# rpng/suo_slam

Measured on AMD Instinct MI355X. Metric: frames/sec (obj-crops/sec) YCB-V 640x480 8-obj; ADD(-S) vs ref, higher is better.
Workload: dtype f32 (2 x fp16 split products)

## Files before the change

### suo_slam_amd/build.py

```python
from __future__ import annotations

import os
import subprocess
import sys

HERE = os.path.dirname(os.path.abspath(__file__))
CSRC = os.path.join(HERE, "csrc")
LIB = os.path.join(HERE, "libsuo_hip.so")
SOURCES = ["capi.hip", "net.hip", "net_weights.hip", "conv.hip", "conv_wino.hip", "conv_wino_x3.hip", "conv_small.hip", "stem_x3.hip", "res_small.hip", "res_small_x3.hip", "gemm_persist.hip", "gemm_bf16x3.hip", "misc.hip", "calibrate.hip", "pnp.hip", "lm.hip", "lm_big.hip", "lm_cam.hip", "lm_cam2.hip", "lm_frame.hip", "lm_frame2.hip", "lm_dist.hip", "pose_cov.hip", "pose_cov_graph.hip", "resid_stats.hip", "track_cov.hip", "ba_comm.hip", "pnp_api.hip", "ba_stage.hip", "ba_api.hip", "ba_ctx.hip", "ba_drive.hip", "cov_stage.hip", "pose_cov_api.hip", "track_cov_api.hip", "frame_geom.hip", "eval.hip", "eval_bop.hip", "eval_nees.hip", "eval_nees_api.hip", "raster.hip", "eval_vsd.hip", "gt_info.hip", "gt_info_api.hip", "slam_score.hip", "slam_vote.hip"]
HIPCC = os.environ.get("HIPCC", "/opt/rocm/bin/hipcc")
FLAGS = ["--offload-arch=gfx950", "-O3", "-std=c++17", "-fPIC", "-ffp-contract=off"]


def _stale(target, deps):
    if not os.path.exists(target):
        return True
    t = os.path.getmtime(target)
    return any(os.path.getmtime(d) > t for d in deps)


def build(force: bool = False, verbose: bool = True) -> str:
    srcs = [os.path.join(CSRC, s) for s in SOURCES if os.path.exists(os.path.join(CSRC, s))]
    hdrs = [os.path.join(CSRC, f) for f in os.listdir(CSRC) if f.endswith(".h")]
    hdrs.append(os.path.join(os.path.dirname(HERE), "include", "suo_hip.h"))
    objs = []
    procs = []
    for src in srcs:
        obj = src[:-4] + ".o"
        objs.append(obj)
        deps = [src] + hdrs
        if src.endswith("lm_big.hip"):
            deps.append(os.path.join(CSRC, "lm.hip"))
        if force or _stale(obj, deps):
            cmd = [HIPCC] + FLAGS + ["-c", src, "-o", obj]
            if verbose:
                print(" ".join(cmd), flush=True)
            procs.append((src, subprocess.Popen(cmd)))
    for src, p in procs:
        if p.wait() != 0:
            raise RuntimeError(f"hipcc failed on {src}")
    if force or procs or _stale(LIB, objs):
        cmd = [HIPCC, "--offload-arch=gfx950", "-shared", "-fPIC", "-o", LIB] + objs + ["-ldl"]
        if verbose:
            print(" ".join(cmd), flush=True)
        subprocess.check_call(cmd)
    return LIB


if __name__ == "__main__":
    build(force="--force" in sys.argv)
    print(LIB)
```

### suo_slam_amd/csrc/conv_wino_x3.hip

```cpp
#include <string.h>

#include "bf16x3.h"
#include "f16x2.h"
#include "buffer_ops.h"
#include "suo_internal.h"
#include "tune.h"

namespace suo {

typedef float x_f32x4 __attribute__((ext_vector_type(4)));
typedef float x_f32x16 __attribute__((ext_vector_type(16)));
typedef unsigned x_u32x2 __attribute__((ext_vector_type(2)));
typedef unsigned x_u32x4 __attribute__((ext_vector_type(4)));
typedef __bf16 x_bf16x8 __attribute__((ext_vector_type(8)));
typedef _Float16 x_f16x8 __attribute__((ext_vector_type(8)));

__device__ __forceinline__ x_f32x16 x_mfma32(float a, float b, x_f32x16 c) { return __builtin_amdgcn_mfma_f32_32x32x2f32(a, b, c, 0, 0, 0); }
__device__ __forceinline__ int x_acc_row(int r, int lane) { return (r & 3) + 8 * (r >> 2) + 4 * (lane >> 5); }

__device__ __forceinline__ x_f32x4 x_sub4(x_f32x4 a, x_f32x4 b) { return a - b; }
__device__ __forceinline__ x_f32x4 x_add4(x_f32x4 a, x_f32x4 b) { return a + b; }
__device__ __forceinline__ void x_add16(x_f32x16& z, const x_f32x16& t) { z += t; }
__device__ __forceinline__ void x_sub16(x_f32x16& z, const x_f32x16& t) { z -= t; }

constexpr int X_CK = 16, X_PKH = 20, X_TH = 8, X_TW = 16, X_IH = 10, X_IW = 18, X_NPIX = X_IH * X_IW;

void pack_wino_weight_bf16x3(const float* W, int N, int C, int Np, int Cp, const float* out_scale, uint16_t* out) {
    static const double G[4][3] = {{1, 0, 0}, {0.5, 0.5, 0.5}, {0.5, -0.5, 0.5}, {0, 0, 1}};
    const int NB = Np / 32;
    memset(out, 0, (size_t)Np * Cp * 16 * 3 * sizeof(uint16_t));
    for (int n = 0; n < N; ++n)
        for (int c = 0; c < C; ++c) {
            const float* g = W + ((size_t)n * C + c) * 9;
            const double sc = out_scale ? (double)out_scale[n] : 1.0;
            double Gg[4][3], U[4][4];
            for (int i = 0; i < 4; ++i)
                for (int j = 0; j < 3; ++j) Gg[i][j] = G[i][0] * g[j] + G[i][1] * g[3 + j] + G[i][2] * g[6 + j];
            for (int i = 0; i < 4; ++i)
                for (int j = 0; j < 4; ++j) U[i][j] = (Gg[i][0] * G[j][0] + Gg[i][1] * G[j][1] + Gg[i][2] * G[j][2]) * sc;
            const int chunk = c / X_CK, cc = c % X_CK, nb = n / 32, lane = (cc / 8) * 32 + (n % 32), e = cc % 8;
            for (int comp = 0; comp < 16; ++comp) {
                uint16_t t[3];
                s3_split_host((float)(comp >= 12 ? -U[comp >> 2][comp & 3] : U[comp >> 2][comp & 3]), t);
                for (int p = 0; p < 3; ++p) out[((((size_t)(chunk * 16 + comp) * NB + nb) * 3 + p) * 64 + lane) * 8 + e] = t[p];
            }
        }
}

void pack_tail_weight_bf16x3(const float* W3, int N2, int K, uint16_t* out) {
    const int NB = N2 / 32;
    for (int n = 0; n < N2; ++n)
        for (int k = 0; k < K; ++k) {
            const int ks = k / 16, kk = k % 16, lane = (kk / 8) * 32 + (n % 32), e = kk % 8, nb = n / 32;
            uint16_t t[3];
            s3_split_host(W3[(size_t)n * K + k], t);
            for (int p = 0; p < 3; ++p) out[((((size_t)(ks * NB + nb) * 3 + p) * 64 + lane) * 8) + e] = t[p];
        }
}

void pack_wino_weight_f16x2(const float* W, int N, int C, int Np, int Cp, const float* out_scale, uint16_t* out, float* oscale_out) {
    static const double G[4][3] = {{1, 0, 0}, {0.5, 0.5, 0.5}, {0.5, -0.5, 0.5}, {0, 0, 1}};
    const int NB = Np / 32;
    memset(out, 0, (size_t)Np * Cp * 16 * 2 * sizeof(uint16_t));
    for (int n = 0; n < Np; ++n) oscale_out[n] = ldexpf(1.f, -S2_XSHIFT);
    float* Un = (float*)malloc((size_t)C * 16 * sizeof(float));
    for (int n = 0; n < N; ++n) {
        float mx = 0.f;
        for (int c = 0; c < C; ++c) {
            const float* g = W + ((size_t)n * C + c) * 9;
            const double sc = out_scale ? (double)out_scale[n] : 1.0;
            double Gg[4][3];
            for (int i = 0; i < 4; ++i)
                for (int j = 0; j < 3; ++j) Gg[i][j] = G[i][0] * g[j] + G[i][1] * g[3 + j] + G[i][2] * g[6 + j];
            for (int i = 0; i < 4; ++i)
                for (int j = 0; j < 4; ++j) {
                    const float u = (float)((Gg[i][0] * G[j][0] + Gg[i][1] * G[j][1] + Gg[i][2] * G[j][2]) * sc);
                    Un[c * 16 + i * 4 + j] = i == 3 ? -u : u;
                    mx = fmaxf(mx, fabsf(u));
                }
        }
        const int t = s2_row_shift(mx);
        oscale_out[n] = ldexpf(1.f, -(t + S2_XSHIFT));
        for (int c = 0; c < C; ++c) {
            const int chunk = c / X_CK, cc = c % X_CK, nb = n / 32, lane = (cc / 8) * 32 + (n % 32), e = cc % 8;
            for (int comp = 0; comp < 16; ++comp) {
                uint16_t h[2];
                s2_split_host(ldexpf(Un[c * 16 + comp], t), h);
                for (int p = 0; p < 2; ++p) out[((((size_t)(chunk * 16 + comp) * NB + nb) * 2 + p) * 64 + lane) * 8 + e] = h[p];
            }
        }
    }
    free(Un);
}

void pack_tail_weight_f16x2(const float* W3, int N2, int K, uint16_t* out, float* oscale_out) { pack_gemm_weight_f16x2(W3, N2, K, out, oscale_out); }

template <bool FUSE, bool UP = false, bool TX3 = false, int NT = 4, int NP = 3, bool NEXT = false, bool W8 = false>
__global__ __launch_bounds__(W8 ? 512 : 256) __attribute__((amdgpu_waves_per_eu(2))) void wino3x3_x3_kernel(const ConvArgs a) {
    static_assert(NT == 4 || (NT == 2 && !FUSE), "64-channel form: plain convolution only");
    static_assert(!W8 || (NT == 4 && NP == 2 && !NEXT && (TX3 || !FUSE)), "eight waves: the fp16 form of the 128-channel kernel, without the next block's conv1");
    constexpr int NTHR = W8 ? 512 : 256;
    static_assert(!NEXT || (FUSE && TX3 && NP == 2), "the next block's conv1 rides on the fp16 tail");
    static_assert(NP == 3 || !FUSE || TX3, "the fp16 form's tail runs on the fp16 pipe");
    constexpr int HSZ = X_NPIX * X_PKH;
    constexpr int VROW = 16;
    constexpr int VPL = 16 * 32 * VROW;
    constexpr int VFLOATS = NP * VPL / 2;
    constexpr int TAILF = NP * 8 * (64 * 32 + 32) / 4;
    constexpr int SFLOATS = W8 ? (2 * HSZ + VFLOATS > TAILF + 8 * 32 * 36 ? 2 * HSZ + VFLOATS : TAILF + 8 * 32 * 36) : 2 * HSZ + VFLOATS;
    __shared__ __attribute__((aligned(16))) float S[SFLOATS];
    float (*Hin)[HSZ] = reinterpret_cast<float (*)[HSZ]>(&S[0]);
    uint16_t* V = reinterpret_cast<uint16_t*>(&S[2 * HSZ]);
    const int tid = threadIdx.x, lane = tid & 63;
    const int w = __builtin_amdgcn_readfirstlane(tid >> 6);
    const int tiles_x = (a.OW + X_TW - 1) / X_TW, tiles_y = (a.OH + X_TH - 1) / X_TH;
    int bid = blockIdx.x;
    if ((gridDim.x & 7) == 0) bid = (bid & 7) * (gridDim.x >> 3) + (bid >> 3);
    const int l = bid / (tiles_x * tiles_y);
    bid -= l * tiles_x * tiles_y;
    const int ty0 = bid / tiles_x, tx0 = bid - ty0 * tiles_x;
    const int oy0 = ty0 * X_TH, ox0 = tx0 * X_TW;
    const int iy0 = oy0 - 1, ix0 = ox0 - 1;
    const int nch = a.C / X_CK;
    const float* in_l = a.in + (size_t)l * a.H * a.W * a.C;
    const __amdgpu_buffer_rsrc_t in_srd = make_srd(in_l, (size_t)a.H * a.W * a.C * sizeof(float));
    const __amdgpu_buffer_rsrc_t w_srd = make_srd(a.Wp, (size_t)a.N * a.C * 16 * NP * sizeof(uint16_t));
    const __amdgpu_buffer_rsrc_t out_srd = make_srd(a.out + (size_t)l * a.OH * a.OW * a.N, (size_t)a.OH * a.OW * a.N * sizeof(float));

    constexpr int NF4 = X_NPIX * 4, NLD = (NF4 + NTHR - 1) / NTHR;
    int avoff[NLD];
#pragma unroll
    for (int i = 0; i < NLD; ++i) {
        const int idx = tid + i * NTHR;
        const int pix = idx >> 2, cc = idx & 3;
        const int py = pix / X_IW, px = pix - py * X_IW;
        const int iy = iy0 + py, ix = ix0 + px;
        const bool ok = idx < NF4 && iy >= 0 && iy < a.H && ix >= 0 && ix < a.W;
        avoff[i] = ok ? ((iy * a.W + ix) * a.C + cc * 4) * 4 : BUF_OOB;
    }
    x_f32x4 areg[NLD];
    auto gload = [&](int c) {
#pragma unroll
        for (int i = 0; i < NLD; ++i) areg[i] = buf_load(in_srd, avoff[i], c * X_CK * 4);
    };
    float dmax = 0.f;
    const float xs = NP == 2 ? s2_xscale(a.xscale) : 1.f;
    auto sstore = [&](int buf) {
#pragma unroll
        for (int i = 0; i < NLD; ++i) {
            const int idx = tid + i * NTHR;
            if constexpr (NP == 2) {
                areg[i] *= xs;
                dmax = s2_track(s2_track(dmax, areg[i][0], areg[i][1]), areg[i][2], areg[i][3]);
            }
            if (idx < NF4) *(x_f32x4*)&Hin[buf][(idx >> 2) * X_PKH + (idx & 3) * 4] = areg[i];
        }
    };
    const int wvoff = lane * 16;
    const int wn = NT == 4 ? (W8 ? (w & 3) : w) : (w & 1), wc = NT == 4 ? (W8 ? (w >> 2) : 0) : (w >> 1);
    constexpr bool HALF = NT == 2 || W8;
    constexpr int NPAIR = HALF ? 4 : 8;
    const int wsbase = wn * NP * 1024;
    auto bload = [&](int gc, x_u32x4 (&b)[NP]) {
        const int g = gc;
#pragma unroll
        for (int p = 0; p < NP; ++p) b[p] = __builtin_bit_cast(x_u32x4, buf_load(w_srd, wvoff + p * 1024, g * (NT * NP * 1024) + wsbase));
    };
    const int tt = tid & 31, tq = (tid >> 5) & 3, th = (tid >> 7) & 1;
    const int tv = __builtin_amdgcn_readfirstlane(tid >> 8);
    const int t_ty = tt >> 3, t_tx = tt & 7;
    const int hbase = ((2 * t_ty + th) * X_IW + 2 * t_tx) * X_PKH + tq * 4;
    const int vbase = tt * VROW + ((((tq >> 1) ^ (((tt >> 2) ^ (tt >> 3)) & 1)) * 8) + (tq & 1) * 4);
    auto vstore = [&](int comp, x_f32x4 v) {
        if constexpr (NP == 2) {
            const unsigned h0 = s2_pack_rn(v[0], v[1]), h1 = s2_pack_rn(v[2], v[3]);
            *(x_u32x2*)&V[comp * 32 * VROW + vbase] = x_u32x2{h0, h1};
            const unsigned l0 = s2_lo_pack(v[0], v[1], h0), l1 = s2_lo_pack(v[2], v[3], h1);
            *(x_u32x2*)&V[VPL + comp * 32 * VROW + vbase] = x_u32x2{l0, l1};
            return;
        }
#pragma unroll
        for (int p = 0; p < 3; ++p) {
            const unsigned q0 = s3_pack_rn(v[0], v[1]), q1 = s3_pack_rn(v[2], v[3]);
            *(x_u32x2*)&V[p * VPL + comp * 32 * VROW + vbase] = x_u32x2{q0, q1};
            if (p < 2) {
                v = x_sub4(v, x_f32x4{s3_lo(q0), s3_hi(q0), s3_lo(q1), s3_hi(q1)});
            }
        }
    };
    const int hother = th ? 0 : 2 * X_IW * X_PKH;
    const float hsign = th ? -1.f : 1.f;
    auto transform = [&](int buf) {
        const float* hs = &Hin[buf][hbase];
        if constexpr (W8) {
            const int xi = tv == 0 ? (th ? 3 : 0) : (th ? 2 : 1);
            x_f32x4 e[4];
#pragma unroll
            for (int c = 0; c < 4; ++c) {
                if (tv == 0) {
                    e[c] = x_sub4(*(const x_f32x4*)(hs + c * X_PKH), *(const x_f32x4*)(hs + (2 * X_IW + c) * X_PKH));
                } else {
                    const x_f32x4 l1 = *(const x_f32x4*)(hs + (X_IW + c) * X_PKH), lx = *(const x_f32x4*)(hs + hother + c * X_PKH);
                    e[c] = x_f32x4{__builtin_fmaf(lx[0], hsign, l1[0]), __builtin_fmaf(lx[1], hsign, l1[1]), __builtin_fmaf(lx[2], hsign, l1[2]), __builtin_fmaf(lx[3], hsign, l1[3])};
                }
            }
            vstore(xi * 4 + 0, x_sub4(e[0], e[2]));
            vstore(xi * 4 + 1, x_add4(e[1], e[2]));
            vstore(xi * 4 + 2, x_sub4(e[2], e[1]));
            vstore(xi * 4 + 3, x_sub4(e[1], e[3]));
            return;
        }
        x_f32x4 L0[4], L1[4], L2[4], Lx[4];
#pragma unroll
        for (int c = 0; c < 4; ++c) {
            L0[c] = *(const x_f32x4*)(hs + c * X_PKH);
            L1[c] = *(const x_f32x4*)(hs + (X_IW + c) * X_PKH);
            L2[c] = *(const x_f32x4*)(hs + (2 * X_IW + c) * X_PKH);
            Lx[c] = *(const x_f32x4*)(hs + hother + c * X_PKH);
        }
        x_f32x4 eA[4], eB[4];
#pragma unroll
        for (int c = 0; c < 4; ++c) {
            eA[c] = x_sub4(L0[c], L2[c]);
            eB[c] = x_f32x4{__builtin_fmaf(Lx[c][0], hsign, L1[c][0]), __builtin_fmaf(Lx[c][1], hsign, L1[c][1]), __builtin_fmaf(Lx[c][2], hsign, L1[c][2]),
                            __builtin_fmaf(Lx[c][3], hsign, L1[c][3])};
        }
        const int xiA = th ? 3 : 0, xiB = th ? 2 : 1;
        vstore(xiA * 4 + 0, x_sub4(eA[0], eA[2]));
        vstore(xiA * 4 + 1, x_add4(eA[1], eA[2]));
        vstore(xiA * 4 + 2, x_sub4(eA[2], eA[1]));
        vstore(xiA * 4 + 3, x_sub4(eA[1], eA[3]));
        vstore(xiB * 4 + 0, x_sub4(eB[0], eB[2]));
        vstore(xiB * 4 + 1, x_add4(eB[1], eB[2]));
        vstore(xiB * 4 + 2, x_sub4(eB[2], eB[1]));
        vstore(xiB * 4 + 3, x_sub4(eB[1], eB[3]));
    };

    x_f32x16 zero16;
#pragma unroll
    for (int r = 0; r < 16; ++r) zero16[r] = 0.f;
    x_f32x16 out[4], Z[8];
#pragma unroll
    for (int p = 0; p < 4; ++p)
#pragma unroll
        for (int r = 0; r < 16; ++r) out[p][r] = 0.f;
#pragma unroll
    for (int p = 0; p < 8; ++p)
#pragma unroll
        for (int r = 0; r < 16; ++r) Z[p][r] = 0.f;
    auto mac6 = [&](x_f32x16& acc, const x_bf16x8 (&f)[NP], const x_u32x4 (&bw)[NP], bool from_zero) {
        if constexpr (NP == 2) {
            constexpr int UI[3] = {0, 1, 0}, UJ[3] = {1, 0, 0};
#pragma unroll
            for (int t = 0; t < 3; ++t)
                acc = __builtin_amdgcn_mfma_f32_32x32x16_f16(__builtin_bit_cast(x_f16x8, f[UI[t]]), __builtin_bit_cast(x_f16x8, bw[UJ[t]]), (t == 0 && from_zero) ? zero16 : acc, 0, 0, 0);
            return;
        }
        constexpr int TI[6] = {0, 1, 2, 0, 1, 0}, TJ[6] = {2, 1, 0, 1, 0, 0};
#pragma unroll
        for (int t = 0; t < 6; ++t)
            acc = __builtin_amdgcn_mfma_f32_32x32x16_bf16(f[TI[t] % NP], __builtin_bit_cast(x_bf16x8, bw[TJ[t] % NP]), (t == 0 && from_zero) ? zero16 : acc, 0, 0, 0);
    };
    auto comp_of = [&](int pair, int which) -> int {
        if (!HALF) return pair < 4 ? (which ? 12 + pair : pair) : (which ? 8 + (pair - 4) : 4 + (pair - 4));
        return wc * 8 + 2 * pair + which;
    };
    const int afoff = (lane & 31) * VROW + (((lane >> 5) ^ (((lane >> 2) ^ (lane >> 3)) & 1)) * 8);
    x_u32x4 bring[2][2][NP];
    gload(0);
    bload(comp_of(0, 0), bring[0][0]);
    bload(comp_of(0, 1), bring[0][1]);
    sstore(0);
    __syncthreads();

#ifdef SUO_WX3_PROF
    long long pt[5] = {0, 0, 0, 0, 0}, p0 = clock64();
#define XPROF(i) do { const long long _t = clock64(); pt[i] += _t - p0; p0 = _t; } while (0)
#else
#define XPROF(i) do { } while (0)
#endif
    for (int c = 0; c < nch; ++c) {
        const int buf = c & 1;
        const bool more = c + 1 < nch;
        if (more) gload(c + 1);
        transform(buf);
        XPROF(0);
        __syncthreads();
        XPROF(1);
        if (more) sstore(buf ^ 1);
        XPROF(2);
#pragma unroll
        for (int pair = 0; pair < NPAIR; ++pair) {
            const int slot = pair & 1;
            {
                const int np = pair + 1 < NPAIR ? pair + 1 : 0, nc = pair + 1 < NPAIR ? c : (more ? c + 1 : c);
                bload(nc * 16 + comp_of(np, 0), bring[slot ^ 1][0]);
                bload(nc * 16 + comp_of(np, 1), bring[slot ^ 1][1]);
            }
            const int ca = comp_of(pair, 0), cb = comp_of(pair, 1);
            x_bf16x8 afa[NP], afb[NP];
#pragma unroll
            for (int p = 0; p < NP; ++p) {
                afa[p] = *(const x_bf16x8*)&V[p * VPL + ca * 32 * VROW + afoff];
                afb[p] = *(const x_bf16x8*)&V[p * VPL + cb * 32 * VROW + afoff];
            }
            __builtin_amdgcn_sched_barrier(0);
            if (HALF) {
                mac6(Z[2 * pair], afa, bring[slot][0], false);
                mac6(Z[2 * pair + 1], afb, bring[slot][1], false);
            } else if (pair < 4) {
                mac6(Z[pair], afa, bring[slot][0], false);
                mac6(Z[4 + pair], afb, bring[slot][1], false);
            } else {
                x_f32x16 ta, tb;
                mac6(ta, afa, bring[slot][0], true);
                mac6(tb, afb, bring[slot][1], true);
                x_add16(Z[pair - 4], ta); x_add16(Z[pair - 4], tb); x_add16(Z[pair], ta); x_sub16(Z[pair], tb);
            }
            __builtin_amdgcn_sched_barrier(0);
        }
        XPROF(3);
        __syncthreads();
        XPROF(4);
    }
#ifdef SUO_WX3_PROF
    if (blockIdx.x == 1000 && (tid & 63) == 0) printf("wave %d cycles: transform %lld  barrier1 %lld  sstore %lld  mfma+fold %lld  barrier2 %lld\n", w, pt[0], pt[1], pt[2], pt[3], pt[4]);
#endif
    if constexpr (NP == 2) s2_raise(a.range_flag, 4.f * dmax);
#pragma unroll
    for (int h = 0; h < 2; ++h) {
        out[2 * h] = Z[4 * h] + Z[4 * h + 1] + Z[4 * h + 2];
        out[2 * h + 1] = Z[4 * h + 1] - Z[4 * h + 2] - Z[4 * h + 3];
    }
    x_f32x16 mine[2];
    if constexpr (W8) {
        static_assert(VFLOATS >= 8 * 16 * 64, "the exchange area is the V planes");
        float* X = &S[2 * HSZ];
        const int pw = (1 - wc) * 4 + wn;
#pragma unroll
        for (int q = 0; q < 2; ++q) {
#pragma unroll
            for (int r = 0; r < 16; ++r) X[(w * 16 + r) * 64 + lane] = wc == 0 ? out[2 + q][r] : out[q][r];
            __syncthreads();
#pragma unroll
            for (int r = 0; r < 16; ++r) mine[q][r] = (wc == 0 ? out[q][r] + out[2 + q][r] : out[2 + q][r] - out[q][r]) + X[(pw * 16 + r) * 64 + lane];
            __syncthreads();
        }
    }

    if constexpr (FUSE && TX3) {
        constexpr int KS_STRIDE = 64 * 32 + 32;
        constexpr int PL_STRIDE = 8 * KS_STRIDE;
        static_assert(NP * PL_STRIDE == TAILF * 4 && NP * PL_STRIDE + (W8 ? 8 : 4) * 32 * 36 * 4 <= SFLOATS * 4, "tail staging must fit the workgroup's LDS");
        constexpr int NJ = W8 ? 1 : 2;
        unsigned char* AP = reinterpret_cast<unsigned char*>(&S[0]);
        float* T = &S[NP * PL_STRIDE / 4] + w * (32 * 36);
        const __amdgpu_buffer_rsrc_t w3_srd = make_srd(a.W3p, (size_t)a.N * a.N2 * NP * sizeof(uint16_t));
        const size_t crop2 = (size_t)a.OH * a.OW * a.N2;
        const __amdgpu_buffer_rsrc_t r_srd = make_srd(a.R + (size_t)l * crop2, crop2 * sizeof(float));
        const __amdgpu_buffer_rsrc_t o2_srd = make_srd(a.out2 + (size_t)l * crop2, crop2 * sizeof(float));
        constexpr bool has_up = UP;
        const __amdgpu_buffer_rsrc_t up_srd = make_srd(has_up ? a.up + (size_t)l * (crop2 / 4) : a.R, has_up ? crop2 / 4 * sizeof(float) : 0);
        const float xs3 = NP == 2 ? s2_xscale(a.xscale3) : 1.f;
        const float b2v = NP == 2 ? a.bias[wn * 32 + (lane & 31)] * xs3 : a.bias[wn * 32 + (lane & 31)];
        const float c2v = NP == 2 ? a.oscale[wn * 32 + (lane & 31)] * xs3 : 1.f;
        float tmax = 0.f;
        const int sbase = (2 * wn + ((lane >> 4) & 1)) * KS_STRIDE + (lane >> 5) * (8 * 32) + ((((lane >> 3) & 1) ^ (lane >> 5)) * 16) + (lane & 7) * 2;
        const int aoff = (lane & 31) * 32 + (((lane >> 5) ^ ((lane >> 3) & 1)) * 16);
        const int w3voff = lane * 16;
        auto b3load = [&](int ks, x_u32x4 (&b)[2][NP]) {
            const int k = ks < 8 ? ks : 7;
#pragma unroll
            for (int j = 0; j < NJ; ++j)
#pragma unroll
                for (int p = 0; p < NP; ++p) b[j][p] = __builtin_bit_cast(x_u32x4, buf_load(w3_srd, w3voff, (((k * 8 + (W8 ? w : 4 * j + w)) * NP) + p) * 1024));
        };
#pragma unroll
        for (int h = 0; h < 2; ++h) {
            x_u32x4 b3[2][2][NP];
            b3load(0, b3[0]);
            if (!W8 || wc == h)
#pragma unroll
            for (int pj = 0; pj < 2; ++pj)
#pragma unroll
                for (int r = 0; r < 16; ++r) {
                    const float cv = W8 ? mine[pj][r] : out[2 * h + pj][r];
                    float v = NP == 2 ? fmaxf(fmaf(cv, c2v, b2v), 0.f) : fmaxf(cv + b2v, 0.f);
                    const int off = sbase + (16 * (r >> 2) + 2 * (r & 3) + pj) * 32;
                    if constexpr (NP == 2) {
                        tmax = fmaxf(tmax, v);
                        const _Float16 hi = (_Float16)v, lo = (_Float16)(v - (float)hi);
                        *reinterpret_cast<_Float16*>(AP + off) = hi;
                        *reinterpret_cast<_Float16*>(AP + PL_STRIDE + off) = lo;
                        continue;
                    }
#pragma unroll
                    for (int p = 0; p < 3; ++p) {
                        const unsigned q = s3_pack_rn(v, v);
                        *reinterpret_cast<uint16_t*>(AP + p * PL_STRIDE + off) = (uint16_t)(q >> 16);
                        if (p < 2) v -= s3_hi(q);
                    }
                }
            __syncthreads();
            x_f32x16 acc2[2][2];
#pragma unroll
            for (int i = 0; i < 2; ++i)
#pragma unroll
                for (int j = 0; j < 2; ++j)
#pragma unroll
                    for (int r = 0; r < 16; ++r) acc2[i][j][r] = 0.f;
#pragma unroll
            for (int ks = 0; ks < 8; ++ks) {
                b3load(ks + 1, b3[(ks + 1) & 1]);
                x_bf16x8 af[2][NP];
#pragma unroll
                for (int i = 0; i < 2; ++i)
#pragma unroll
                    for (int p = 0; p < NP; ++p) af[i][p] = *(const x_bf16x8*)(AP + p * PL_STRIDE + ks * KS_STRIDE + i * 1024 + aoff);
                __builtin_amdgcn_sched_barrier(0);
#pragma unroll
                for (int i = 0; i < 2; ++i)
#pragma unroll
                    for (int j = 0; j < NJ; ++j) mac6(acc2[i][j], af[i], b3[ks & 1][j], false);
                __builtin_amdgcn_sched_barrier(0);
            }
            if constexpr (NEXT) __syncthreads();
            x_f32x16 acc1[2];
            if constexpr (NEXT) {
#pragma unroll
                for (int i = 0; i < 2; ++i) acc1[i] = zero16;
            }
#pragma unroll
            for (int j = 0; j < NJ; ++j) {
#pragma unroll
                for (int i = 0; i < 2; ++i) {
                    const int col = (W8 ? w : 4 * j + w) * 32 + (lane & 7) * 4;
                    const x_f32x4 bv = *(const x_f32x4*)(a.bias3 + col);
                    x_f32x4 osc3 = x_f32x4{1.f, 1.f, 1.f, 1.f};
                    if constexpr (NP == 2) osc3 = *(const x_f32x4*)(a.oscale3 + col);
                    x_f32x4 nsc, nsh;
                    if constexpr (NEXT) { const float nxs = s2_xscale(a.n_xscale); nsc = *(const x_f32x4*)(a.n_scale + col) * nxs; nsh = *(const x_f32x4*)(a.n_shift + col) * nxs; }
                    int off[4];
                    x_f32x4 rv[4], uv[UP ? 4 : 1];
#pragma unroll
                    for (int k = 0; k < 4; ++k) {
                        const int m = 32 * i + (lane >> 3) + 8 * k;
                        const int oy = oy0 + 2 * (m >> 4) + h, ox = ox0 + (m & 15);
                        const bool in = oy < a.OH && ox < a.OW;
                        off[k] = in ? ((oy * a.OW + ox) * a.N2 + col) * 4 : BUF_OOB;
                        rv[k] = buf_load(r_srd, off[k], 0);
                        if constexpr (UP && !NEXT) uv[k] = buf_load(up_srd, in ? (((oy >> 1) * (a.OW >> 1) + (ox >> 1)) * a.N2 + col) * 4 : BUF_OOB, 0);
                    }
#pragma unroll
                    for (int r = 0; r < 16; ++r) T[x_acc_row(r, lane) * 36 + (lane & 31)] = acc2[i][j][r];
                    __builtin_amdgcn_wave_barrier();
#pragma unroll
                    for (int k = 0; k < 4; ++k) {
                        if constexpr (UP && NEXT) {
                            const int m = 32 * i + (lane >> 3) + 8 * k;
                            const int oy = oy0 + 2 * (m >> 4) + h, ox = ox0 + (m & 15);
                            uv[0] = buf_load(up_srd, (oy < a.OH && ox < a.OW) ? (((oy >> 1) * (a.OW >> 1) + (ox >> 1)) * a.N2 + col) * 4 : BUF_OOB, 0);
                        }
                        x_f32x4 o = *(const x_f32x4*)&T[((lane >> 3) + 8 * k) * 36 + (lane & 7) * 4];
                        if constexpr (NP == 2) o *= osc3;
                        o = (o + bv) + rv[k];
                        if constexpr (UP) o += uv[NEXT ? 0 : k];
                        buf_store(o, o2_srd, off[k]);
                        if constexpr (NEXT) {
                            const int m = 32 * i + (lane >> 3) + 8 * k;
                            float xn[4];
#pragma unroll
                            for (int c = 0; c < 4; ++c) xn[c] = fmaxf(fmaf(o[c], nsc[c], nsh[c]), 0.f);
                            tmax = fmaxf(fmaxf(tmax, fmaxf(xn[0], xn[1])), fmaxf(xn[2], xn[3]));
                            const unsigned h0 = s2_pack_rn(xn[0], xn[1]), h1 = s2_pack_rn(xn[2], xn[3]);
                            const unsigned l0 = s2_lo_pack(xn[0], xn[1], h0), l1 = s2_lo_pack(xn[2], xn[3], h1);
                            unsigned char* d = AP + (2 * w + ((lane & 7) >> 2)) * KS_STRIDE + m * 32 + (((((lane & 3) >> 1) ^ ((m >> 3) & 1))) * 16) + (lane & 1) * 8;
                            *reinterpret_cast<x_u32x2*>(d) = x_u32x2{h0, h1};
                            *reinterpret_cast<x_u32x2*>(d + PL_STRIDE) = x_u32x2{l0, l1};
                        }
                    }
                    __builtin_amdgcn_wave_barrier();
                }
                if constexpr (NEXT) {
                    const __amdgpu_buffer_rsrc_t n1_srd = make_srd(a.n_W1, (size_t)128 * 256 * 2 * sizeof(uint16_t));
                    auto n1load = [&](int q, x_u32x4 (&b)[2]) {
                        const int ksg = 8 * j + (q < 8 ? q : 7);
#pragma unroll
                        for (int p = 0; p < 2; ++p) b[p] = __builtin_bit_cast(x_u32x4, buf_load(n1_srd, w3voff + p * 1024, ((ksg * 4 + w) * 2) * 1024));
                    };
                    constexpr int NR = 4;
                    x_u32x4 nb[NR][2];
#pragma unroll
                    for (int q = 0; q < NR - 1; ++q) n1load(q, nb[q]);
                    __syncthreads();
#pragma unroll
                    for (int q = 0; q < 8; ++q) {
                        n1load(q + NR - 1, nb[(q + NR - 1) % NR]);
                        x_bf16x8 af[2][2];
#pragma unroll
                        for (int i = 0; i < 2; ++i)
#pragma unroll
                            for (int p = 0; p < 2; ++p) af[i][p] = *(const x_bf16x8*)(AP + p * PL_STRIDE + q * KS_STRIDE + i * 1024 + aoff);
                        __builtin_amdgcn_sched_barrier(0);
#pragma unroll
                        for (int i = 0; i < 2; ++i) mac6(acc1[i], af[i], nb[q % NR], false);
                        __builtin_amdgcn_sched_barrier(0);
                    }
                    __syncthreads();
                }
            }
            if constexpr (NEXT) {
                const int col = w * 32 + (lane & 7) * 4;
                const x_f32x4 b1 = *(const x_f32x4*)(a.n_b1 + col), o1 = *(const x_f32x4*)(a.n_osc1 + col);
                const size_t cropn = (size_t)a.OH * a.OW * 128;
                const __amdgpu_buffer_rsrc_t n_srd = make_srd(a.n_out + (size_t)l * cropn, cropn * sizeof(float));
#pragma unroll
                for (int i = 0; i < 2; ++i) {
#pragma unroll
                    for (int r = 0; r < 16; ++r) T[x_acc_row(r, lane) * 36 + (lane & 31)] = acc1[i][r];
                    __builtin_amdgcn_wave_barrier();
#pragma unroll
                    for (int k = 0; k < 4; ++k) {
                        const int m = 32 * i + (lane >> 3) + 8 * k;
                        const int oy = oy0 + 2 * (m >> 4) + h, ox = ox0 + (m & 15);
                        x_f32x4 o = *(const x_f32x4*)&T[((lane >> 3) + 8 * k) * 36 + (lane & 7) * 4];
                        o *= o1;
                        o += b1;
#pragma unroll
                        for (int c = 0; c < 4; ++c) o[c] = fmaxf(o[c], 0.f);
                        buf_store(o, n_srd, (oy < a.OH && ox < a.OW) ? ((oy * a.OW + ox) * 128 + col) * 4 : BUF_OOB);
                    }
                    __builtin_amdgcn_wave_barrier();
                }
            }
            if (h == 0 && !NEXT) __syncthreads();
        }
        if constexpr (NP == 2) s2_raise(a.range_flag, tmax);
        return;
    }

    if constexpr (FUSE && !TX3) {
        constexpr int MP = 132;
        static_assert(128 * MP <= 2 * HSZ + VFLOATS, "the conv2 tile must fit the workgroup's LDS");
        float* M2 = &S[0];
        const int wm = w >> 1, wn = w & 1;
        const int NB2 = a.N2 >> 5;
        const __amdgpu_buffer_rsrc_t w3_srd = make_srd(a.W3p, (size_t)a.N * a.N2 * sizeof(float));
        const size_t crop2 = (size_t)a.OH * a.OW * a.N2;
        const __amdgpu_buffer_rsrc_t r_srd = make_srd(a.R + (size_t)l * crop2, crop2 * sizeof(float));
        const __amdgpu_buffer_rsrc_t o2_srd = make_srd(a.out2 + (size_t)l * crop2, crop2 * sizeof(float));
        constexpr bool has_up = UP;
        const __amdgpu_buffer_rsrc_t up_srd = make_srd(has_up ? a.up + (size_t)l * (crop2 / 4) : a.R, has_up ? crop2 / 4 * sizeof(float) : 0);
        const float b2v = a.bias[w * 32 + (lane & 31)];
        const int w3voff = lane * 16;
        auto b3load = [&](int q, x_f32x4(&b)[4]) {
            const int kg = q < 16 ? q : 15;
#pragma unroll
            for (int j = 0; j < 4; ++j) b[j] = buf_load(w3_srd, w3voff, (kg * NB2 + wn * 4 + j) * 1024);
        };
        constexpr int R3 = 3;
        x_f32x4 b3[R3][4];
#pragma unroll
        for (int r = 0; r < R3 - 1; ++r) b3load(r, b3[r]);
#pragma unroll
        for (int p = 0; p < 4; ++p)
#pragma unroll
            for (int r = 0; r < 16; ++r) {
                const int t = x_acc_row(r, lane);
                const int pix = (2 * (t >> 3) + (p >> 1)) * X_TW + 2 * (t & 7) + (p & 1);
                M2[pix * MP + w * 32 + (lane & 31)] = fmaxf(out[p][r] + b2v, 0.f);
            }
        __syncthreads();
        x_f32x16 acc2[2][4];
#pragma unroll
        for (int i = 0; i < 2; ++i)
#pragma unroll
            for (int j = 0; j < 4; ++j)
#pragma unroll
                for (int r = 0; r < 16; ++r) acc2[i][j][r] = 0.f;
        const float* ms = M2 + ((wm * 2) * 32 + (lane & 31)) * MP + (lane >> 5) * 4;
#pragma unroll
        for (int q = 0; q < 16; ++q) {
            b3load(q + R3 - 1, b3[(q + R3 - 1) % R3]);
            __builtin_amdgcn_sched_barrier(0);
            x_f32x4 af[2];
#pragma unroll
            for (int i = 0; i < 2; ++i) af[i] = *(const x_f32x4*)(ms + i * 32 * MP + q * 8);
#pragma unroll
            for (int t = 0; t < 4; ++t)
#pragma unroll
                for (int i = 0; i < 2; ++i)
#pragma unroll
                    for (int j = 0; j < 4; ++j) acc2[i][j] = x_mfma32(af[i][t], b3[q % R3][j][t], acc2[i][j]);
            __builtin_amdgcn_sched_barrier(0);
        }
        __syncthreads();
#pragma unroll
        for (int i = 0; i < 2; ++i)
#pragma unroll
            for (int j = 0; j < 4; ++j) {
                float* T = M2 + w * (32 * 36);
                const int col = (wn * 4 + j) * 32 + (lane & 7) * 4;
                const x_f32x4 bv = *(const x_f32x4*)(a.bias3 + col);
                int off[4];
                x_f32x4 rv[4], uv[UP ? 4 : 1];
#pragma unroll
                for (int k = 0; k < 4; ++k) {
                    const int pp = (wm * 2 + i) * 32 + (lane >> 3) + 8 * k;
                    const int oy = oy0 + pp / X_TW, ox = ox0 + pp % X_TW;
                    const bool in = oy < a.OH && ox < a.OW;
                    off[k] = in ? ((oy * a.OW + ox) * a.N2 + col) * 4 : BUF_OOB;
                    rv[k] = buf_load(r_srd, off[k], 0);
                    if constexpr (UP) uv[k] = buf_load(up_srd, in ? (((oy >> 1) * (a.OW >> 1) + (ox >> 1)) * a.N2 + col) * 4 : BUF_OOB, 0);
                }
#pragma unroll
                for (int r = 0; r < 16; ++r) T[x_acc_row(r, lane) * 36 + (lane & 31)] = acc2[i][j][r];
                __builtin_amdgcn_wave_barrier();
#pragma unroll
                for (int k = 0; k < 4; ++k) {
                    x_f32x4 o = (*(const x_f32x4*)&T[((lane >> 3) + 8 * k) * 36 + (lane & 7) * 4] + bv) + rv[k];
                    if constexpr (UP) o += uv[k];
                    buf_store(o, o2_srd, off[k]);
                }
                __builtin_amdgcn_wave_barrier();
            }
        return;
    }

    if constexpr (NT == 2 || W8) {
        if constexpr (NT == 2) {
            float* X = &S[2 * HSZ];
#pragma unroll
            for (int q = 0; q < 2; ++q)
#pragma unroll
                for (int r = 0; r < 16; ++r) X[((w * 2 + q) * 16 + r) * 64 + lane] = wc == 0 ? out[2 + q][r] : out[q][r];
            __syncthreads();
            const int pw = (1 - wc) * 2 + wn;
#pragma unroll
            for (int q = 0; q < 2; ++q)
#pragma unroll
                for (int r = 0; r < 16; ++r)
                    mine[q][r] = (wc == 0 ? out[q][r] + out[2 + q][r] : out[2 + q][r] - out[q][r]) + X[((pw * 2 + q) * 16 + r) * 64 + lane];
            __syncthreads();
        }
        float* T = &S[2 * HSZ] + w * (32 * 36);
        const int col = wn * 32 + (lane & 7) * 4;
        const x_f32x4 bv = *(const x_f32x4*)(a.bias + col);
        x_f32x4 osc = x_f32x4{1.f, 1.f, 1.f, 1.f};
        if constexpr (NP == 2) osc = *(const x_f32x4*)(a.oscale + col);
#pragma unroll
        for (int q = 0; q < 2; ++q) {
            const int p = 2 * wc + q, pi = p >> 1, pj = p & 1;
#pragma unroll
            for (int r = 0; r < 16; ++r) T[x_acc_row(r, lane) * 36 + (lane & 31)] = mine[q][r];
            __builtin_amdgcn_wave_barrier();
#pragma unroll
            for (int k = 0; k < 4; ++k) {
                const int t = (lane >> 3) + 8 * k;
                const int oy = oy0 + 2 * (t >> 3) + pi, ox = ox0 + 2 * (t & 7) + pj;
                x_f32x4 o = *(const x_f32x4*)&T[t * 36 + (lane & 7) * 4];
                if constexpr (NP == 2) o *= osc;
                o += bv;
                if (a.relu) {
#pragma unroll
                    for (int z = 0; z < 4; ++z) o[z] = fmaxf(o[z], 0.f);
                }
                buf_store(o, out_srd, (oy < a.OH && ox < a.OW) ? ((oy * a.OW + ox) * a.N + col) * 4 : BUF_OOB);
            }
            __builtin_amdgcn_wave_barrier();
        }
        return;
    }

    float* T = &S[2 * HSZ] + w * (32 * 36);
    const int col = w * 32 + (lane & 7) * 4;
    const x_f32x4 bv = *(const x_f32x4*)(a.bias + col);
    x_f32x4 osc = x_f32x4{1.f, 1.f, 1.f, 1.f};
    if constexpr (NP == 2) osc = *(const x_f32x4*)(a.oscale + col);
#pragma unroll
    for (int p = 0; p < 4; ++p) {
        const int pi = p >> 1, pj = p & 1;
#pragma unroll
        for (int r = 0; r < 16; ++r) T[x_acc_row(r, lane) * 36 + (lane & 31)] = out[p][r];
        __builtin_amdgcn_wave_barrier();
#pragma unroll
        for (int k = 0; k < 4; ++k) {
            const int t = (lane >> 3) + 8 * k;
            const int oy = oy0 + 2 * (t >> 3) + pi, ox = ox0 + 2 * (t & 7) + pj;
            x_f32x4 o = *(const x_f32x4*)&T[t * 36 + (lane & 7) * 4];
            if constexpr (NP == 2) o *= osc;
            o += bv;
            if (a.relu) {
#pragma unroll
                for (int q = 0; q < 4; ++q) o[q] = fmaxf(o[q], 0.f);
            }
            buf_store(o, out_srd, (oy < a.OH && ox < a.OW) ? ((oy * a.OW + ox) * a.N + col) * 4 : BUF_OOB);
        }
        __builtin_amdgcn_wave_barrier();
    }
}

bool conv3x3_wino_f16x2_w8(long tiles) {
    static const long upto = SUO_TUNE("SUO_WINO_W8_TILES", 256);
    return tiles > 0 && tiles <= upto && env_switch("SUO_WINO_W8", 1) != 0;
}

template <int NP>
static int launch_wino_split(const ConvArgs& a, hipStream_t s) {
    if (NP == 2 && (!a.oscale || !a.range_flag)) { suo_set_error("conv3x3_wino_f16x2: oscale / range_flag missing"); return SUO_ERR_ARG; }
    if (a.OH == a.H && a.OW == a.W && a.N == 64 && a.C == 64) {
        const int tiles64 = ((a.OW + X_TW - 1) / X_TW) * ((a.OH + X_TH - 1) / X_TH) * a.L;
        hipLaunchKernelGGL((wino3x3_x3_kernel<false, false, false, 2, NP>), dim3(tiles64), dim3(256), 0, s, a);
        SUO_HIP_CHECK(hipGetLastError());
        return SUO_OK;
    }
    if (a.OH != a.H || a.OW != a.W || a.N != 128 || a.C != 128) {
        suo_set_error("conv3x3_wino_x3: unsupported shape H=%d W=%d C=%d N=%d", a.H, a.W, a.C, a.N);
        return SUO_ERR_ARG;
    }
    const int tiles = ((a.OW + X_TW - 1) / X_TW) * ((a.OH + X_TH - 1) / X_TH) * a.L;
    if (NP == 2 && conv3x3_wino_f16x2_w8(tiles)) hipLaunchKernelGGL((wino3x3_x3_kernel<false, false, false, 4, 2, false, true>), dim3(tiles), dim3(512), 0, s, a);
    else hipLaunchKernelGGL((wino3x3_x3_kernel<false, false, false, 4, NP>), dim3(tiles), dim3(256), 0, s, a);
    SUO_HIP_CHECK(hipGetLastError());
    return SUO_OK;
}
int launch_conv3x3_wino_x3(const ConvArgs& a, hipStream_t s) { return launch_wino_split<3>(a, s); }
int launch_conv3x3_wino_f16x2(const ConvArgs& a, hipStream_t s) { return launch_wino_split<2>(a, s); }

int launch_conv3x3_wino_f16x2_fused(const ConvArgs& a, hipStream_t s) {
    if (a.OH != a.H || a.OW != a.W || a.N != 128 || a.C != 128 || a.N2 != 256 || !a.W3p || !a.bias3 || !a.R || !a.out2 || !a.oscale || !a.oscale3 || !a.range_flag) {
        suo_set_error("conv3x3_wino_f16x2_fused: unsupported shape C=%d N=%d N2=%d", a.C, a.N, a.N2);
        return SUO_ERR_ARG;
    }
    const int tiles = ((a.OW + X_TW - 1) / X_TW) * ((a.OH + X_TH - 1) / X_TH) * a.L;
    if (a.n_W1) {
        if (!a.n_scale || !a.n_shift || !a.n_osc1 || !a.n_b1 || !a.n_out) { suo_set_error("conv3x3_wino_f16x2_fused: incomplete next-block arguments"); return SUO_ERR_ARG; }
        if (a.up) { suo_set_error("conv3x3_wino_f16x2_fused: the next block's conv1 cannot ride on a tail with an up-sampled addend"); return SUO_ERR_ARG; }
        hipLaunchKernelGGL((wino3x3_x3_kernel<true, false, true, 4, 2, true>), dim3(tiles), dim3(256), 0, s, a);
    } else if (conv3x3_wino_f16x2_w8(tiles)) {
        if (a.up) hipLaunchKernelGGL((wino3x3_x3_kernel<true, true, true, 4, 2, false, true>), dim3(tiles), dim3(512), 0, s, a);
        else hipLaunchKernelGGL((wino3x3_x3_kernel<true, false, true, 4, 2, false, true>), dim3(tiles), dim3(512), 0, s, a);
    } else if (a.up) hipLaunchKernelGGL((wino3x3_x3_kernel<true, true, true, 4, 2>), dim3(tiles), dim3(256), 0, s, a);
    else hipLaunchKernelGGL((wino3x3_x3_kernel<true, false, true, 4, 2>), dim3(tiles), dim3(256), 0, s, a);
    SUO_HIP_CHECK(hipGetLastError());
    return SUO_OK;
}

int launch_conv3x3_wino_x3_fused(const ConvArgs& a, hipStream_t s) {
    if (a.OH != a.H || a.OW != a.W || a.N != 128 || a.C != 128 || a.N2 != 256 || !a.W3p || !a.bias3 || !a.R || !a.out2) {
        suo_set_error("conv3x3_wino_x3_fused: unsupported shape C=%d N=%d N2=%d", a.C, a.N, a.N2);
        return SUO_ERR_ARG;
    }
    const int tiles = ((a.OW + X_TW - 1) / X_TW) * ((a.OH + X_TH - 1) / X_TH) * a.L;
    if (a.w3_bf16x3) {
        if (a.up) hipLaunchKernelGGL((wino3x3_x3_kernel<true, true, true>), dim3(tiles), dim3(256), 0, s, a);
        else hipLaunchKernelGGL((wino3x3_x3_kernel<true, false, true>), dim3(tiles), dim3(256), 0, s, a);
    } else {
        if (a.up) hipLaunchKernelGGL((wino3x3_x3_kernel<true, true, false>), dim3(tiles), dim3(256), 0, s, a);
        else hipLaunchKernelGGL((wino3x3_x3_kernel<true, false, false>), dim3(tiles), dim3(256), 0, s, a);
    }
    SUO_HIP_CHECK(hipGetLastError());
    return SUO_OK;
}

}
```

Before: 1405.

## Load Winograd input halo directly into LDS via buffer_load LDS-DMA

```diff
diff --git a/suo_slam_amd/build.py b/suo_slam_amd/build.py
--- a/suo_slam_amd/build.py
+++ b/suo_slam_amd/build.py
@@ -7,7 +7,7 @@
 HERE = os.path.dirname(os.path.abspath(__file__))
 CSRC = os.path.join(HERE, "csrc")
 LIB = os.path.join(HERE, "libsuo_hip.so")
-SOURCES = ["capi.hip", "net.hip", "net_weights.hip", "conv.hip", "conv_wino.hip", "conv_wino_x3.hip", "conv_small.hip", "stem_x3.hip", "res_small.hip", "res_small_x3.hip", "gemm_persist.hip", "gemm_bf16x3.hip", "misc.hip", "calibrate.hip", "pnp.hip", "lm.hip", "lm_big.hip", "lm_cam.hip", "lm_cam2.hip", "lm_frame.hip", "lm_frame2.hip", "lm_dist.hip", "pose_cov.hip", "pose_cov_graph.hip", "resid_stats.hip", "track_cov.hip", "ba_comm.hip", "pnp_api.hip", "ba_stage.hip", "ba_api.hip", "ba_ctx.hip", "ba_drive.hip", "cov_stage.hip", "pose_cov_api.hip", "track_cov_api.hip", "frame_geom.hip", "eval.hip", "eval_bop.hip", "eval_nees.hip", "eval_nees_api.hip", "raster.hip", "eval_vsd.hip", "gt_info.hip", "gt_info_api.hip", "slam_score.hip", "slam_vote.hip"]
+SOURCES = ["capi.hip", "net.hip", "net_weights.hip", "conv.hip", "conv_wino.hip", "conv_wino_x3.hip", "conv_wino_x3_dma.hip", "conv_small.hip", "stem_x3.hip", "res_small.hip", "res_small_x3.hip", "gemm_persist.hip", "gemm_bf16x3.hip", "misc.hip", "calibrate.hip", "pnp.hip", "lm.hip", "lm_big.hip", "lm_cam.hip", "lm_cam2.hip", "lm_frame.hip", "lm_frame2.hip", "lm_dist.hip", "pose_cov.hip", "pose_cov_graph.hip", "resid_stats.hip", "track_cov.hip", "ba_comm.hip", "pnp_api.hip", "ba_stage.hip", "ba_api.hip", "ba_ctx.hip", "ba_drive.hip", "cov_stage.hip", "pose_cov_api.hip", "track_cov_api.hip", "frame_geom.hip", "eval.hip", "eval_bop.hip", "eval_nees.hip", "eval_nees_api.hip", "raster.hip", "eval_vsd.hip", "gt_info.hip", "gt_info_api.hip", "slam_score.hip", "slam_vote.hip"]
 HIPCC = os.environ.get("HIPCC", "/opt/rocm/bin/hipcc")
 FLAGS = ["--offload-arch=gfx950", "-O3", "-std=c++17", "-fPIC", "-ffp-contract=off"]
 
@@ -31,6 +31,8 @@
         deps = [src] + hdrs
         if src.endswith("lm_big.hip"):
             deps.append(os.path.join(CSRC, "lm.hip"))
+        if src.endswith("conv_wino_x3_dma.hip"):
+            deps.append(os.path.join(CSRC, "conv_wino_x3.hip"))
         if force or _stale(obj, deps):
             cmd = [HIPCC] + FLAGS + ["-c", src, "-o", obj]
             if verbose:
diff --git a/suo_slam_amd/csrc/conv_wino_x3.hip b/suo_slam_amd/csrc/conv_wino_x3.hip
--- a/suo_slam_amd/csrc/conv_wino_x3.hip
+++ b/suo_slam_amd/csrc/conv_wino_x3.hip
@@ -25,6 +25,7 @@
 
 constexpr int X_CK = 16, X_PKH = 20, X_TH = 8, X_TW = 16, X_IH = 10, X_IW = 18, X_NPIX = X_IH * X_IW;
 
+#ifndef SUO_WX3_DMA_TU
 void pack_wino_weight_bf16x3(const float* W, int N, int C, int Np, int Cp, const float* out_scale, uint16_t* out) {
     static const double G[4][3] = {{1, 0, 0}, {0.5, 0.5, 0.5}, {0.5, -0.5, 0.5}, {0, 0, 1}};
     const int NB = Np / 32;
@@ -94,10 +95,12 @@
 }
 
 void pack_tail_weight_f16x2(const float* W3, int N2, int K, uint16_t* out, float* oscale_out) { pack_gemm_weight_f16x2(W3, N2, K, out, oscale_out); }
-
-template <bool FUSE, bool UP = false, bool TX3 = false, int NT = 4, int NP = 3, bool NEXT = false, bool W8 = false>
+#endif
+
+template <bool FUSE, bool UP = false, bool TX3 = false, int NT = 4, int NP = 3, bool NEXT = false, bool W8 = false, bool DMA = false>
 __global__ __launch_bounds__(W8 ? 512 : 256) __attribute__((amdgpu_waves_per_eu(2))) void wino3x3_x3_kernel(const ConvArgs a) {
     static_assert(NT == 4 || (NT == 2 && !FUSE), "64-channel form: plain convolution only");
+    static_assert(!DMA || (NP == 2 && !W8), "halo by LDS-DMA: the four-wave fp16 form");
     static_assert(!W8 || (NT == 4 && NP == 2 && !NEXT && (TX3 || !FUSE)), "eight waves: the fp16 form of the 128-channel kernel, without the next block's conv1");
     constexpr int NTHR = W8 ? 512 : 256;
     static_assert(!NEXT || (FUSE && TX3 && NP == 2), "the next block's conv1 rides on the fp16 tail");
@@ -128,16 +131,36 @@
     const __amdgpu_buffer_rsrc_t out_srd = make_srd(a.out + (size_t)l * a.OH * a.OW * a.N, (size_t)a.OH * a.OW * a.N * sizeof(float));
 
     constexpr int NF4 = X_NPIX * 4, NLD = (NF4 + NTHR - 1) / NTHR;
+    constexpr int HP = DMA ? 16 : X_PKH;
+    static_assert(!DMA || (NLD == 3 && NLD * NTHR * 4 <= HSZ), "LDS-DMA staging: three 1 KiB pieces per wave inside a halo buffer");
     int avoff[NLD];
 #pragma unroll
     for (int i = 0; i < NLD; ++i) {
         const int idx = tid + i * NTHR;
-        const int pix = idx >> 2, cc = idx & 3;
+        const int pix = idx >> 2;
         const int py = pix / X_IW, px = pix - py * X_IW;
+        const int cc = DMA ? (idx & 3) ^ ((py >> 1) & 3) : idx & 3;
         const int iy = iy0 + py, ix = ix0 + px;
         const bool ok = idx < NF4 && iy >= 0 && iy < a.H && ix >= 0 && ix < a.W;
         avoff[i] = ok ? ((iy * a.W + ix) * a.C + cc * 4) * 4 : BUF_OOB;
     }
+    const unsigned lds_w = __builtin_amdgcn_readfirstlane((unsigned)(size_t)&S[0]) + w * 1024;
+    auto dma = [&](int c, int buf) {
+        if constexpr (DMA) {
+            const unsigned d0 = lds_w + buf * (HSZ * 4), d1 = d0 + NTHR * 16, d2 = d0 + 2 * NTHR * 16;
+            const int soff = c * X_CK * 4;
+            unsigned keep;
+            asm volatile("s_mov_b32 %0, m0\n\t"
+                         "s_nop 4\n\t"
+                         "s_mov_b32 m0, %5\n\ts_nop 0\n\tbuffer_load_dwordx4 %1, %4, %8 offen lds\n\t"
+                         "s_mov_b32 m0, %6\n\ts_nop 0\n\tbuffer_load_dwordx4 %2, %4, %8 offen lds\n\t"
+                         "s_mov_b32 m0, %7\n\ts_nop 0\n\tbuffer_load_dwordx4 %3, %4, %8 offen lds\n\t"
+                         "s_mov_b32 m0, %0"
+                         : "=&s"(keep)
+                         : "v"(avoff[0]), "v"(avoff[NLD > 1 ? 1 : 0]), "v"(avoff[NLD > 2 ? 2 : 0]), "s"(in_srd), "s"(d0), "s"(d1), "s"(d2), "s"(soff)
+                         : "memory");
+        }
+    };
     x_f32x4 areg[NLD];
     auto gload = [&](int c) {
 #pragma unroll
@@ -154,6 +177,13 @@
                 dmax = s2_track(s2_track(dmax, areg[i][0], areg[i][1]), areg[i][2], areg[i][3]);
             }
             if (idx < NF4) *(x_f32x4*)&Hin[buf][(idx >> 2) * X_PKH + (idx & 3) * 4] = areg[i];
+        }
+    };
+    auto dtrack = [&](int buf) {
+#pragma unroll
+        for (int i = 0; i < NLD; ++i) {
+            const x_f32x4 v = *(const x_f32x4*)&Hin[buf][(tid + i * NTHR) * 4];
+            dmax = s2_track(s2_track(dmax, v[0], v[1]), v[2], v[3]);
         }
     };
     const int wvoff = lane * 16;
@@ -169,7 +199,8 @@
     const int tt = tid & 31, tq = (tid >> 5) & 3, th = (tid >> 7) & 1;
     const int tv = __builtin_amdgcn_readfirstlane(tid >> 8);
     const int t_ty = tt >> 3, t_tx = tt & 7;
-    const int hbase = ((2 * t_ty + th) * X_IW + 2 * t_tx) * X_PKH + tq * 4;
+    const int hbase = ((2 * t_ty + th) * X_IW + 2 * t_tx) * HP + (DMA ? (tq ^ t_ty) : tq) * 4;
+    const int hbase1 = DMA ? ((2 * t_ty + th) * X_IW + 2 * t_tx) * HP + (tq ^ ((t_ty + 1) & 3)) * 4 : hbase;
     const int vbase = tt * VROW + ((((tq >> 1) ^ (((tt >> 2) ^ (tt >> 3)) & 1)) * 8) + (tq & 1) * 4);
     auto vstore = [&](int comp, x_f32x4 v) {
         if constexpr (NP == 2) {
@@ -188,7 +219,7 @@
             }
         }
     };
-    const int hother = th ? 0 : 2 * X_IW * X_PKH;
+    const int hother = th ? 0 : 2 * X_IW * HP;
     const float hsign = th ? -1.f : 1.f;
     auto transform = [&](int buf) {
         const float* hs = &Hin[buf][hbase];
@@ -210,13 +241,16 @@
             vstore(xi * 4 + 3, x_sub4(e[1], e[3]));
             return;
         }
+        const float* hs2 = &Hin[buf][hbase1];
+        const float* hs1 = th ? hs2 : hs;
+        const float* hsx = th ? hs : hs2;
         x_f32x4 L0[4], L1[4], L2[4], Lx[4];
 #pragma unroll
         for (int c = 0; c < 4; ++c) {
-            L0[c] = *(const x_f32x4*)(hs + c * X_PKH);
-            L1[c] = *(const x_f32x4*)(hs + (X_IW + c) * X_PKH);
-            L2[c] = *(const x_f32x4*)(hs + (2 * X_IW + c) * X_PKH);
-            Lx[c] = *(const x_f32x4*)(hs + hother + c * X_PKH);
+            L0[c] = *(const x_f32x4*)(hs + c * HP);
+            L1[c] = *(const x_f32x4*)(hs1 + (X_IW + c) * HP);
+            L2[c] = *(const x_f32x4*)(hs2 + (2 * X_IW + c) * HP);
+            Lx[c] = *(const x_f32x4*)(hsx + hother + c * HP);
         }
         x_f32x4 eA[4], eB[4];
 #pragma unroll
@@ -224,6 +258,7 @@
             eA[c] = x_sub4(L0[c], L2[c]);
             eB[c] = x_f32x4{__builtin_fmaf(Lx[c][0], hsign, L1[c][0]), __builtin_fmaf(Lx[c][1], hsign, L1[c][1]), __builtin_fmaf(Lx[c][2], hsign, L1[c][2]),
                             __builtin_fmaf(Lx[c][3], hsign, L1[c][3])};
+            if constexpr (DMA) { eA[c] *= xs; eB[c] *= xs; }
         }
         const int xiA = th ? 3 : 0, xiB = th ? 2 : 1;
         vstore(xiA * 4 + 0, x_sub4(eA[0], eA[2]));
@@ -267,10 +302,21 @@
     };
     const int afoff = (lane & 31) * VROW + (((lane >> 5) ^ (((lane >> 2) ^ (lane >> 3)) & 1)) * 8);
     x_u32x4 bring[2][2][NP];
-    gload(0);
+    if constexpr (DMA) {
+#pragma unroll
+        for (int i = 0; i < NLD; ++i)
+            if (avoff[i] == BUF_OOB) {
+                *(x_f32x4*)&Hin[0][(tid + i * NTHR) * 4] = x_f32x4{0.f, 0.f, 0.f, 0.f};
+                *(x_f32x4*)&Hin[1][(tid + i * NTHR) * 4] = x_f32x4{0.f, 0.f, 0.f, 0.f};
+            }
+        dma(0, 0);
+    } else {
+        gload(0);
+    }
     bload(comp_of(0, 0), bring[0][0]);
     bload(comp_of(0, 1), bring[0][1]);
-    sstore(0);
+    if constexpr (DMA) asm volatile("s_waitcnt vmcnt(0)" ::: "memory");
+    else sstore(0);
     __syncthreads();
 
 #ifdef SUO_WX3_PROF
@@ -282,12 +328,16 @@
     for (int c = 0; c < nch; ++c) {
         const int buf = c & 1;
         const bool more = c + 1 < nch;
-        if (more) gload(c + 1);
+        if (more) {
+            if constexpr (DMA) dma(c + 1, buf ^ 1);
+            else gload(c + 1);
+        }
         transform(buf);
+        if constexpr (DMA) dtrack(buf);
         XPROF(0);
         __syncthreads();
         XPROF(1);
-        if (more) sstore(buf ^ 1);
+        if (more && !DMA) sstore(buf ^ 1);
         XPROF(2);
 #pragma unroll
         for (int pair = 0; pair < NPAIR; ++pair) {
@@ -320,9 +370,11 @@
             __builtin_amdgcn_sched_barrier(0);
         }
         XPROF(3);
+        if constexpr (DMA) asm volatile("s_waitcnt vmcnt(4)" ::: "memory");
         __syncthreads();
         XPROF(4);
     }
+    if constexpr (DMA) dmax *= xs;
 #ifdef SUO_WX3_PROF
     if (blockIdx.x == 1000 && (tid & 63) == 0) printf("wave %d cycles: transform %lld  barrier1 %lld  sstore %lld  mfma+fold %lld  barrier2 %lld\n", w, pt[0], pt[1], pt[2], pt[3], pt[4]);
 #endif
@@ -700,16 +752,22 @@
     }
 }
 
+#ifndef SUO_WX3_DMA_TU
 bool conv3x3_wino_f16x2_w8(long tiles) {
     static const long upto = SUO_TUNE("SUO_WINO_W8_TILES", 256);
     return tiles > 0 && tiles <= upto && env_switch("SUO_WINO_W8", 1) != 0;
 }
+
+bool conv3x3_wino_f16x2_dma() { return env_switch("SUO_WINO_HALO_DMA", 1) != 0; }
+int launch_conv3x3_wino_f16x2_dma(const ConvArgs& a, hipStream_t s, int tiles);
+int launch_conv3x3_wino_f16x2_fused_dma(const ConvArgs& a, hipStream_t s, int tiles);
 
 template <int NP>
 static int launch_wino_split(const ConvArgs& a, hipStream_t s) {
     if (NP == 2 && (!a.oscale || !a.range_flag)) { suo_set_error("conv3x3_wino_f16x2: oscale / range_flag missing"); return SUO_ERR_ARG; }
     if (a.OH == a.H && a.OW == a.W && a.N == 64 && a.C == 64) {
         const int tiles64 = ((a.OW + X_TW - 1) / X_TW) * ((a.OH + X_TH - 1) / X_TH) * a.L;
+        if (NP == 2 && conv3x3_wino_f16x2_dma()) return launch_conv3x3_wino_f16x2_dma(a, s, tiles64);
         hipLaunchKernelGGL((wino3x3_x3_kernel<false, false, false, 2, NP>), dim3(tiles64), dim3(256), 0, s, a);
         SUO_HIP_CHECK(hipGetLastError());
         return SUO_OK;
@@ -720,6 +778,7 @@
     }
     const int tiles = ((a.OW + X_TW - 1) / X_TW) * ((a.OH + X_TH - 1) / X_TH) * a.L;
     if (NP == 2 && conv3x3_wino_f16x2_w8(tiles)) hipLaunchKernelGGL((wino3x3_x3_kernel<false, false, false, 4, 2, false, true>), dim3(tiles), dim3(512), 0, s, a);
+    else if (NP == 2 && conv3x3_wino_f16x2_dma()) return launch_conv3x3_wino_f16x2_dma(a, s, tiles);
     else hipLaunchKernelGGL((wino3x3_x3_kernel<false, false, false, 4, NP>), dim3(tiles), dim3(256), 0, s, a);
     SUO_HIP_CHECK(hipGetLastError());
     return SUO_OK;
@@ -733,14 +792,17 @@
         return SUO_ERR_ARG;
     }
     const int tiles = ((a.OW + X_TW - 1) / X_TW) * ((a.OH + X_TH - 1) / X_TH) * a.L;
+    const bool dma = conv3x3_wino_f16x2_dma();
     if (a.n_W1) {
         if (!a.n_scale || !a.n_shift || !a.n_osc1 || !a.n_b1 || !a.n_out) { suo_set_error("conv3x3_wino_f16x2_fused: incomplete next-block arguments"); return SUO_ERR_ARG; }
         if (a.up) { suo_set_error("conv3x3_wino_f16x2_fused: the next block's conv1 cannot ride on a tail with an up-sampled addend"); return SUO_ERR_ARG; }
+        if (dma) return launch_conv3x3_wino_f16x2_fused_dma(a, s, tiles);
         hipLaunchKernelGGL((wino3x3_x3_kernel<true, false, true, 4, 2, true>), dim3(tiles), dim3(256), 0, s, a);
     } else if (conv3x3_wino_f16x2_w8(tiles)) {
         if (a.up) hipLaunchKernelGGL((wino3x3_x3_kernel<true, true, true, 4, 2, false, true>), dim3(tiles), dim3(512), 0, s, a);
         else hipLaunchKernelGGL((wino3x3_x3_kernel<true, false, true, 4, 2, false, true>), dim3(tiles), dim3(512), 0, s, a);
-    } else if (a.up) hipLaunchKernelGGL((wino3x3_x3_kernel<true, true, true, 4, 2>), dim3(tiles), dim3(256), 0, s, a);
+    } else if (dma) return launch_conv3x3_wino_f16x2_fused_dma(a, s, tiles);
+    else if (a.up) hipLaunchKernelGGL((wino3x3_x3_kernel<true, true, true, 4, 2>), dim3(tiles), dim3(256), 0, s, a);
     else hipLaunchKernelGGL((wino3x3_x3_kernel<true, false, true, 4, 2>), dim3(tiles), dim3(256), 0, s, a);
     SUO_HIP_CHECK(hipGetLastError());
     return SUO_OK;
@@ -763,4 +825,20 @@
     return SUO_OK;
 }
 
-}
+#else
+int launch_conv3x3_wino_f16x2_dma(const ConvArgs& a, hipStream_t s, int tiles) {
+    if (a.N == 64) hipLaunchKernelGGL((wino3x3_x3_kernel<false, false, false, 2, 2, false, false, true>), dim3(tiles), dim3(256), 0, s, a);
+    else hipLaunchKernelGGL((wino3x3_x3_kernel<false, false, false, 4, 2, false, false, true>), dim3(tiles), dim3(256), 0, s, a);
+    SUO_HIP_CHECK(hipGetLastError());
+    return SUO_OK;
+}
+int launch_conv3x3_wino_f16x2_fused_dma(const ConvArgs& a, hipStream_t s, int tiles) {
+    if (a.n_W1) hipLaunchKernelGGL((wino3x3_x3_kernel<true, false, true, 4, 2, true, false, true>), dim3(tiles), dim3(256), 0, s, a);
+    else if (a.up) hipLaunchKernelGGL((wino3x3_x3_kernel<true, true, true, 4, 2, false, false, true>), dim3(tiles), dim3(256), 0, s, a);
+    else hipLaunchKernelGGL((wino3x3_x3_kernel<true, false, true, 4, 2, false, false, true>), dim3(tiles), dim3(256), 0, s, a);
+    SUO_HIP_CHECK(hipGetLastError());
+    return SUO_OK;
+}
+#endif
+
+}
diff --git a/suo_slam_amd/csrc/conv_wino_x3_dma.hip b/suo_slam_amd/csrc/conv_wino_x3_dma.hip
--- /dev/null
+++ b/suo_slam_amd/csrc/conv_wino_x3_dma.hip
@@ -0,0 +1,2 @@
+#define SUO_WX3_DMA_TU 1
+#include "conv_wino_x3.hip"
```

Result: faster. 1423, median of 6 (+1.3%).
